# ysnrkdm/subproc

Measured on AMD Instinct MI355X. Metric: env-steps/sec (batched self-play), higher is better.
Workload: dtype u64

## Files before the change

### subproc_amd/csrc/othello.hip

```cpp
#include <hip/hip_runtime.h>
#include <stdint.h>
#include <stdlib.h>

#include <algorithm>
#include <climits>
#include <cmath>
#include <atomic>
#include <mutex>

#include "../../include/othello.h"
#include "bitboard.hpp"
#include "td_skey.hpp"

#define OTH_VERSION "subproc_amd 0.1.0 gfx950"

namespace {

using namespace oth;

constexpr u64 OPEN_BLACK = 0x0000000810000000ull;
constexpr u64 OPEN_WHITE = 0x0000001008000000ull;
constexpr int kBlock = 256;

constexpr u64 GOLDEN64 = 0x9E3779B97F4A7C15ull;
__host__ __device__ __forceinline__ u64 mix64(u64 z) {
    z = (z ^ (z >> 30)) * 0xBF58476D1CE4E5B9ull;
    z = (z ^ (z >> 27)) * 0x94D049BB133111EBull;
    return z ^ (z >> 31);
}
__device__ __forceinline__ u64 game_key(u64 S, u64 g) { return mix64(S + g * GOLDEN64); }
constexpr u32 LCG_MUL = 0x915F77F5u;
struct GameRng {
    u32 state, inc;
    __device__ __forceinline__ void init(u64 key) {
        state = (u32)key;
        inc = (u32)(key >> 32) | 1u;
    }
    __device__ __forceinline__ u32 pick(u32 n) {
        state = state * LCG_MUL + inc;
        return __umulhi(state, n);
    }
};
__device__ __forceinline__ u32 pick_legal(u64 legal, GameRng& rng, const uint8_t* kth_tab) {
    const u32 c_lo = __popc((u32)legal);
    return kth_bit_tab(legal, rng.pick(c_lo + __popc((u32)(legal >> 32))), c_lo, kth_tab);
}


__constant__ u64 kRegionMasks[8] = {0x8100000000000081ull, 0x4281000000008142ull, 0x0042000000004200ull,
                                    0x2400810000810024ull, 0x1800008181000018ull, 0x003C424242423C00ull,
                                    0x0000240000240000ull, 0x0000183C3C180000ull};

constexpr int kEvalRow = 12;
constexpr int kEvalTable = OTH_EVAL_PHASES * kEvalRow;
struct EvalWeights {
    int8_t w[OTH_EVAL_WEIGHTS];
};
__device__ __forceinline__ u32 eval_shard(u32 discs) { return discs ? (min(discs, 64u) - 1u) >> 4 : 0u; }
__device__ __forceinline__ void eval_weights_to_lds(const EvalWeights& ew, int* w_s) {
    for (int e = threadIdx.x; e < OTH_EVAL_PHASES * kEvalRow; e += blockDim.x) {
        const int r = e / kEvalRow, c = e % kEvalRow;
        w_s[e] = c < OTH_EVAL_FEATURES ? (int)ew.w[r * OTH_EVAL_FEATURES + c] : 0;
    }
}
__device__ __forceinline__ int eval_mul(int w, int c) { return __mul24(w, c); }
__device__ __forceinline__ int eval_linear(const int* w, u64 mine, u64 mob) {
    int v = eval_mul(w[0], (int)__popcll(mob));
#pragma unroll
    for (int k = 0; k < 8; k++) v += eval_mul(w[1 + k], (int)__popcll(and2(mine, kRegionMasks[k])));
    return v;
}

template <int POLICY>
__device__ __forceinline__ const int* child_row(u64 P, u64 O, const int* w_tab) {
    if (POLICY != OTH_POLICY_EVAL) return w_tab;
    return w_tab + kEvalRow * eval_shard((u32)__popcll(P | O) + 1u);
}
template <int POLICY>
__device__ __forceinline__ u32 child_key(u64 P, u64 O, const RunSets& s, u32 sq, const u64* rays, const int* row) {
    place(P, O, flips_rays(sq, s, rays));
    if (POLICY == OTH_POLICY_GREEDY) return ((u32)__popcll(moves(O, P)) << 6) | sq;
    int w[OTH_EVAL_FEATURES];
#pragma unroll
    for (int j = 0; j < OTH_EVAL_FEATURES; j++) w[j] = row[j];
    const int v = eval_linear(w, P, moves<789>(P, O));
    return ((u32)((1 << 20) - v) << 6) | sq;
}

template <int POLICY>
__device__ __forceinline__ u32 lane_choose(const Position& pos, u64 P, u64 O, const u64* rays, const int* w_tab) {
    u32 best = 0xFFFFFFFFu;
    u64 legal = pos.legal;
    const RunSets s = run_sets_parent(P, pos);
    const int* row = child_row<POLICY>(P, O, w_tab);
    while (legal) {
        const u32 sq = (u32)__builtin_ctzll(legal);
        legal &= legal - 1;
        best = min(best, child_key<POLICY>(P, O, s, sq, rays, row));
    }
    return best & 63u;
}

struct CoopWave {
    u64 rec[64][10];
    u64 legal[64];
    u32 best[64];
};
__device__ __forceinline__ void wave_sync() {
    __builtin_amdgcn_fence(__ATOMIC_SEQ_CST, "wavefront");
    __builtin_amdgcn_wave_barrier();
}
static_assert(sizeof(Runs) == 8 * sizeof(u64), "parent record: P, O, Runs");
__device__ __forceinline__ void load_parent(const u64* r, u64& P, u64& O, RunSets& s) {
    P = r[0];
    O = r[1];
    s.r = *reinterpret_cast<const Runs*>(r + 2);
    s.P = P;
    s.rP = 0;
}
__device__ __forceinline__ u32 wave_incl_scan(u32 x) {
    x += (u32)__builtin_amdgcn_update_dpp(0, (int)x, 0x111, 0xf, 0xf, false);
    x += (u32)__builtin_amdgcn_update_dpp(0, (int)x, 0x112, 0xf, 0xf, false);
    x += (u32)__builtin_amdgcn_update_dpp(0, (int)x, 0x114, 0xf, 0xf, false);
    x += (u32)__builtin_amdgcn_update_dpp(0, (int)x, 0x118, 0xf, 0xf, false);
    x += (u32)__builtin_amdgcn_update_dpp(0, (int)x, 0x142, 0xa, 0xf, false);
    x += (u32)__builtin_amdgcn_update_dpp(0, (int)x, 0x143, 0xc, 0xf, false);
    return x;
}
template <int POLICY>
__device__ u32 coop_choose(bool need, u64 P, u64 O, u32 tbl, const Position& pos, CoopWave& cw, const u64* rays,
                           const int* w_s, const uint8_t* kth_tab, u32 lane, u32 cap) {
    auto publish = [&] {
        u64* r = cw.rec[lane];
        r[0] = P;
        r[1] = O;
        Runs rs = run_sets_parent(P, pos).r;
        if (POLICY == OTH_POLICY_EVAL) rs.A1 |= (u64)(tbl & 1u);
        *reinterpret_cast<Runs*>(r + 2) = rs;
    };
    constexpr bool kFirst = POLICY == OTH_POLICY_GREEDY;
    if (kFirst && need) publish();
    if (cap == 0) return need ? lane_choose<POLICY>(pos, P, O, rays, w_s + (tbl ? kEvalTable : 0)) : 64u;
    const u64 legal = need ? pos.legal : 0ull;
    const u32 cnt = (u32)__popcll(legal);
    const u32 incl = wave_incl_scan(cnt);
    const u32 T = (u32)__builtin_amdgcn_readlane((int)incl, 63);
    const u32 R = (T + 63u) >> 6;
    cw.legal[lane] = legal;
    if (need) {
        if (!kFirst) publish();
        cw.best[lane] = 0xFFFFFFFFu;
    }
    const u32 t0 = R * lane, cnt_mine = t0 < T ? min(R, T - t0) : 0u;
    const u32 excl = incl - cnt;
    const u64 with_moves = __ballot(cnt != 0);
    u32 p = 0;
#pragma unroll
    for (u32 step = 32; step >= 1; step >>= 1)
        if ((u32)__shfl((int)excl, (int)(p + step)) <= t0) p += step;
    const u32 k0 = t0 - (u32)__shfl((int)excl, (int)p);
    wave_sync();
    u64 m = 0, Pp = 0, Op = 0;
    RunSets ps = {};
    const int* row = w_s;
// ... 72 lines not shown
    if (o.ret >= 0) o.t = black ? OTH_WHITE : OTH_BLACK;
    return o;
}

__global__ __launch_bounds__(kBlock) void legal_kernel(const u64* __restrict__ boards,
                                                       const uint8_t* __restrict__ turn, u64* __restrict__ legal,
                                                       int64_t n) {
    const int64_t i = (int64_t)blockIdx.x * kBlock + threadIdx.x;
    if (i >= n) return;
    const ulonglong2 b = reinterpret_cast<const ulonglong2*>(boards)[i];
    legal[i] = legal_any(b.x, b.y, turn[i]);
}

__device__ __forceinline__ void step_board(int64_t i, ulonglong2 b, u32 t, u32 mvc, u64* boards_out, uint8_t* turn_out,
                                           u64* __restrict__ flips_out,
                                           u64* __restrict__ legal_next, int8_t* __restrict__ ret_out,
                                           uint8_t* __restrict__ nturn) {
    u64 nb, nw, f = 0, lg = 0;
    u32 t_out;
    int r = -1;
    if (t == OTH_BLACK || t == OTH_WHITE) {
        const bool black = t == OTH_BLACK;
        u64 P = black ? b.x : b.y;
        u64 O = black ? b.y : b.x;
        if (mvc == OTH_PASS) {
            r = 0;
        } else if (mvc < 64) {
            const u64 mv = 1ull << mvc;
            if (!((P | O) & mv)) {
                f = flips_carry(mvc, P, O);
                if (f) {
                    r = __popcll(f);
                    P = or3(P, f, mv);
                    O = andn(O, f);
                }
            }
        }
        const bool moved = r >= 0;
        t_out = moved ? (t ^ 3u) : t;
        if (legal_next) {
            const u64 nP = moved ? O : P, nO = moved ? P : O;
            lg = moves(nP, nO);
        }
        nb = black ? P : O;
        nw = black ? O : P;
    } else {
        const StepOut o = put_s_any(b.x, b.y, t, mvc);
        nb = o.bl;
        nw = o.wh;
        f = o.flips;
        r = o.ret;
        t_out = o.t;
        if (legal_next) lg = legal_any(nb, nw, t_out);
    }
    if (legal_next) __builtin_nontemporal_store(lg, legal_next + i);
    if (boards_out) {
        __builtin_nontemporal_store(nb, boards_out + 2 * i);
        __builtin_nontemporal_store(nw, boards_out + 2 * i + 1);
    }
    if (turn_out) __builtin_nontemporal_store((uint8_t)t_out, turn_out + i);
    if (flips_out) __builtin_nontemporal_store(f, flips_out + i);
    if (ret_out) __builtin_nontemporal_store((int8_t)r, ret_out + i);
    if (nturn && r >= 0) nturn[i] = (uint8_t)(nturn[i] + 1);
}

constexpr int kStepPerThread = 1;
__global__ __launch_bounds__(kBlock) void step_kernel(const u64* boards_in, const uint8_t* turn_in,
                                                      const uint8_t* __restrict__ move, u64* boards_out,
                                                      uint8_t* turn_out, u64* __restrict__ flips_out,
                                                      u64* __restrict__ legal_next, int8_t* __restrict__ ret_out,
                                                      uint8_t* __restrict__ nturn, int64_t n) {
    const int64_t i0 = (int64_t)blockIdx.x * kBlock + threadIdx.x, stride = (int64_t)gridDim.x * kBlock;
    ulonglong2 b[kStepPerThread];
    u32 t[kStepPerThread], mvc[kStepPerThread];
#pragma unroll
    for (int j = 0; j < kStepPerThread; j++) {
        const int64_t i = i0 + j * stride;
        if (i < n) {
            b[j] = reinterpret_cast<const ulonglong2*>(boards_in)[i];
            t[j] = turn_in[i];
            mvc[j] = move[i];
            asm volatile("" ::"v"(t[j]), "v"(mvc[j]));
        }
    }
#pragma unroll
    for (int j = 0; j < kStepPerThread; j++) {
        const int64_t i = i0 + j * stride;
        if (i < n) step_board(i, b[j], t[j], mvc[j], boards_out, turn_out, flips_out, legal_next, ret_out, nturn);
    }
}

__device__ __forceinline__ bool step_on_board(int64_t x, int64_t d, int k, int64_t& out) {
    int64_t t;
    return !__builtin_mul_overflow(d, (int64_t)k, &t) && !__builtin_add_overflow(x, t, &out) && out >= 0 && out < 8;
}
__global__ __launch_bounds__(kBlock) void hands_kernel(const u64* __restrict__ own, const u64* __restrict__ hostile,
                                                       const int64_t* __restrict__ xs, const int64_t* __restrict__ ys,
                                                       const int64_t* __restrict__ dxs,
                                                       const int64_t* __restrict__ dys,
                                                       uint8_t* __restrict__ count, int64_t n) {
    const int64_t i = (int64_t)blockIdx.x * kBlock + threadIdx.x;
    if (i >= n) return;
    const u64 mine = own[i], opp = hostile[i];
    const int64_t x = xs[i], y = ys[i], dx = dxs[i], dy = dys[i];
    int run = 0;
    for (int k = 1; k < 9; k++) {
        int64_t nx, ny;
        const bool on = step_on_board(x, dx, k, nx) && step_on_board(y, dy, k, ny);
        const u64 bit = on ? 1ull << (nx + 8 * ny) : 0ull;
        if (opp & bit) {
            run = k;
        } else {
            if (!(mine & bit)) run = 0;
            break;
        }
    }
    count[i] = (uint8_t)run;
}

__global__ __launch_bounds__(kBlock) void result_kernel(const u64* __restrict__ boards, uint8_t* __restrict__ nb,
                                                        uint8_t* __restrict__ nw, int8_t* __restrict__ diff,
                                                        uint8_t* __restrict__ terminal, int64_t n) {
    const int64_t i = (int64_t)blockIdx.x * kBlock + threadIdx.x;
    if (i >= n) return;
    const ulonglong2 b = reinterpret_cast<const ulonglong2*>(boards)[i];
    const int cb = __popcll(b.x), cw = __popcll(b.y);
    if (nb) nb[i] = (uint8_t)cb;
    if (nw) nw[i] = (uint8_t)cw;
    if (diff) diff[i] = (int8_t)(cb - cw);
    if (terminal) terminal[i] = (moves(b.x, b.y) == 0 && moves(b.y, b.x) == 0) ? 1 : 0;
}


struct RolloutArgs {
    const u64* start;
    const uint8_t* start_turn;
    u64 seed_state;
    u64 game_id0;
    int n_random;
    u64* final_boards;
    int8_t* diff;
    uint8_t* plies;
    uint8_t* moves;
    long long* hist;
    int64_t n;
    unsigned long long* work;
    u64 last_ticket;
    u32 coop_cap;
    EvalWeights ew[2];
    u32 n_rand_a, n_rand_b;
    int swap;
    uint8_t* a_black;
    u32 handoff_k;
};

constexpr u32 kHandoffK = 16;
constexpr u32 kHandoffKMax = 16;
constexpr int kPoolCap = 64 + (int)kHandoffKMax;
struct Parked {
    u64 P, O;
    u32 state, inc;
    u32 g;
    u32 bits;
};
static_assert(sizeof(Parked) == 32, "two 16-B LDS accesses per parked game");
constexpr u64 kParkedGame = ~0ull;

constexpr int kRecStride = OTH_MOVES_STRIDE + 4;
constexpr int kRecWaveBytes = 64 * kRecStride;
constexpr size_t rec_stage_bytes(int policy, bool record) {
    return record && policy == OTH_POLICY_RANDOM ? (size_t)(kBlock / 64) * kRecWaveBytes : 0;
}

constexpr int kRandomFillOrder = 789;
constexpr int rollout_waves_per_simd(int policy) { return policy == OTH_POLICY_GREEDY ? 5 : 4; }
template <int POLICY, bool RECORD, bool RUNNER = false>
__global__ __launch_bounds__(kBlock, rollout_waves_per_simd(POLICY)) void rollout_kernel(RolloutArgs a) {
    __shared__ unsigned long long hist_s[OTH_HIST_BINS];
    __shared__ uint8_t kth_tab[256 * 8];
    __shared__ u64 rays[kTabRows * 64];
    __shared__ int w_s[POLICY == OTH_POLICY_EVAL ? 2 * kEvalTable : 1];
    __shared__ CoopWave coop[POLICY == OTH_POLICY_RANDOM ? 1 : kBlock / 64];
    constexpr bool kPool = POLICY == OTH_POLICY_RANDOM && !RECORD && !RUNNER;
    __shared__ Parked pool_s[kPool ? kBlock / 64 : 1][kPool ? kPoolCap : 1];
    for (int k = threadIdx.x; k < OTH_HIST_BINS; k += kBlock) hist_s[k] = 0;
    kth_table_init(kth_tab);
    ray_table_init(rays);
    if (POLICY == OTH_POLICY_EVAL) {
        eval_weights_to_lds(a.ew[0], w_s);
        eval_weights_to_lds(a.ew[1], w_s + kEvalTable);
    }
    __syncthreads();

    const int lane = lane_id();
    const u64 n = (u64)a.n;
    u64 plies_sum = 0;
    constexpr bool kRecStage = RECORD && POLICY == OTH_POLICY_RANDOM;
    extern __shared__ u32 rec_dyn[];
    uint8_t* const rec_wave = reinterpret_cast<uint8_t*>(rec_dyn) + (threadIdx.x >> 6) * kRecWaveBytes;
    uint8_t* const rec_row = rec_wave + lane * kRecStride;

    Parked* const pool = pool_s[kPool ? threadIdx.x >> 6 : 0];
    u32 parked = 0;
    bool exhausted = false;
    (void)pool;
    (void)exhausted;
    for (;;) {
        bool from_pool = false;
        u64 base = 0;
        if (kPool && parked >= 64u) {
            from_pool = true;
        } else if (!kPool || !exhausted) {
            if (lane == 0) {
                base = atomicAdd(a.work, 64ull);
                if (base == a.last_ticket) atomicExch(a.work, 0ull);
            }
            base = __shfl(base, 0);
            if (base >= n) {
                if (!kPool || parked == 0u) break;
                exhausted = true;
                from_pool = true;
            }
        } else {
            if (parked == 0u) break;
            from_pool = true;
        }

        u64 g = base + lane;
        bool active = !from_pool && g < n;
        u64 P = OPEN_BLACK, O = OPEN_WHITE;
        u32 side = OTH_BLACK, ply = 0;
        bool passed = false;
        GameRng rng;
        if (active) {
            rng.init(game_key(a.seed_state, a.game_id0 + g));
            if (a.start) {
                const ulonglong2 s0 = reinterpret_cast<const ulonglong2*>(a.start)[g];
                side = a.start_turn ? a.start_turn[g] : OTH_BLACK;
                side = side == OTH_WHITE ? OTH_WHITE : OTH_BLACK;
                P = side == OTH_BLACK ? s0.x : s0.y;
                O = side == OTH_BLACK ? s0.y : s0.x;
            }
            if (RECORD && !kRecStage) {
                uint4* mrec = reinterpret_cast<uint4*>(a.moves + g * OTH_MOVES_STRIDE);
#pragma unroll
                for (int q = 0; q < OTH_MOVES_STRIDE / 16; q++) mrec[q] = make_uint4(~0u, ~0u, ~0u, ~0u);
            }
        }
        if constexpr (kRecStage) {
#pragma unroll
            for (int q = 0; q < OTH_MOVES_STRIDE / 4; q++) reinterpret_cast<u32*>(rec_row)[q] = ~0u;
        }
        auto rec_put = [&](u32 i, uint8_t code) {
            if (i >= OTH_MOVES_STRIDE) return;
            if constexpr (kRecStage) rec_row[i] = code;
            else a.moves[g * OTH_MOVES_STRIDE + i] = code;
        };

        if constexpr (POLICY == OTH_POLICY_RANDOM) {
            bool b0 = side == OTH_BLACK;
            u32 discs0 = RECORD ? 0u : (u32)__popcll(P | O);
            u32 npass = 0;
            if (kPool && from_pool) {
                const u32 take = min(parked, 64u);
                active = (u32)lane < take;
                if (active) {
                    const Parked e = pool[parked - take + lane];
                    P = e.P;
                    O = e.O;
                    rng.state = e.state;
                    rng.inc = e.inc;
                    g = e.g;
                    b0 = e.bits & 1u;
                    passed = (e.bits >> 1) & 1u;
                    discs0 = (e.bits >> 2) & 0x7fu;
                    npass = e.bits >> 9;
                }
                parked -= take;
            }
            const u32 hand_k = __builtin_amdgcn_readfirstlane(kPool && !from_pool ? a.handoff_k : 0u);
            const u32 parked0 = __builtin_amdgcn_readfirstlane(parked);
            (void)hand_k;
            (void)parked0;
            auto ply_of = [&](u64& X, u64& Y) -> bool {
                Position pos;
                analyse<kRandomFillOrder>(X, Y, pos);
                const u64 legal = pos.legal;
                const u32 c_lo = __popc((u32)legal), nl = c_lo + __popc((u32)(legal >> 32));
                if (nl == 0) {
                    if (passed || (X | Y) == ~0ull) {
                        if (passed) npass--;
                        return true;
                    }
                    if (RECORD) rec_put(npass, OTH_PASS);
                    passed = true;
                    npass++;
                    return false;
                }
                passed = false;
                const u32 off = kth_bit_off(legal, rng.pick(nl), c_lo, kth_tab);
                const u64* col = ray_col(rays, off);
                const Flips f = flips_col(col[kRayRows * 64], run_sets(X, pos), col);
                if (RECORD) {
                    rec_put(npass, (uint8_t)(off >> 3));
                    npass++;
                }
                place(X, Y, f);
                return false;
            };
            if (active) {
                for (;;) {
                    if (ply_of(P, O)) break;
                    if (ply_of(O, P)) break;
                    if (kPool) {
                        const u64 live = __ballot(1);
                        if ((u32)__popcll(live) <= hand_k) {
                            const u32 rank = __builtin_amdgcn_mbcnt_hi((u32)(live >> 32),
                                                                       __builtin_amdgcn_mbcnt_lo((u32)live, 0u));
                            pool[parked0 + rank] = Parked{P, O, rng.state, rng.inc, (u32)g,
                                                          (u32)b0 | (u32)passed << 1 | discs0 << 2 | npass << 9};
                            g = kParkedGame;
                            break;
                        }
                    }
                }
            }
            if (kPool) {
                const u64 pm = __ballot(active && g == kParkedGame);
                parked = parked0 + (u32)__popcll(pm);
                if (g == kParkedGame) active = false;
            }
            if (active) {
                const u32 ply = RECORD ? npass : (u32)__popcll(P | O) - discs0 + npass;
                if (RECORD) rec_put(ply, 0xFF);
                const u64 bl = b0 ? P : O, wh = b0 ? O : P;
                const int d = __popcll(bl) - __popcll(wh);
                if (a.final_boards) reinterpret_cast<ulonglong2*>(a.final_boards)[g] = make_ulonglong2(bl, wh);
                if (a.diff) a.diff[g] = (int8_t)d;
                if (a.plies) a.plies[g] = (uint8_t)ply;
                atomicAdd(&hist_s[d + 64], 1ull);
                atomicAdd(&hist_s[d > 0 ? 129 : (d < 0 ? 130 : 131)], 1ull);
                plies_sum += ply;
            }
        } else {
            u32 rem_b = 0, rem_w = 0, tbl_black = 0;
            if (RUNNER && active) {
                const bool ab = !(a.swap && rng.pick(2) == 1u);
                rem_b = ab ? a.n_rand_a : a.n_rand_b;
                rem_w = ab ? a.n_rand_b : a.n_rand_a;
                tbl_black = ab ? 0u : 1u;
                if (a.a_black) a.a_black[g] = (uint8_t)ab;
            }
            while (__ballot(active)) {
                bool moving = false, choose = false;
                u32 sq = 0;
                Position pos;
                if (active) {
                    analyse(P, O, pos);
                    const u64 legal = pos.legal;
                    if (legal == 0) {
                        if (passed || (P | O) == ~0ull) {
                            const u64 bl = side == OTH_BLACK ? P : O, wh = side == OTH_BLACK ? O : P;
                            const int d = __popcll(bl) - __popcll(wh);
                            u64 gt = g;
                            if (POLICY == OTH_POLICY_GREEDY) asm volatile("" : "+v"(gt));
                            if (a.final_boards)
                                reinterpret_cast<ulonglong2*>(a.final_boards)[gt] = make_ulonglong2(bl, wh);
                            if (a.diff) a.diff[gt] = (int8_t)d;
                            if (a.plies) a.plies[gt] = (uint8_t)ply;
                            atomicAdd(&hist_s[d + 64], 1ull);
                            atomicAdd(&hist_s[d > 0 ? 129 : (d < 0 ? 130 : 131)], 1ull);
                            if (POLICY == OTH_POLICY_GREEDY) atomicAdd(&hist_s[132], (unsigned long long)ply);
                            else plies_sum += ply;
                            active = false;
                        } else {
                            passed = true;
                            const u64 t = P;
                            P = O;
                            O = t;
                            side ^= 3u;
                        }
                    } else {
                        if (passed) {
                            if (RECORD) rec_put(ply, OTH_PASS);
                            ply++;
                            passed = false;
                            if (RUNNER) {
                                const u32 rx = side == OTH_BLACK ? rem_w : rem_b;
                                if (rx) (void)rng.pick(rx);
                            }
                        }
                        moving = true;
                        if (RUNNER) {
                            const u32 r = side == OTH_BLACK ? rem_b : rem_w;
                            if (r && rng.pick(r) == 0u) {
                                sq = pick_legal(legal, rng, kth_tab);
                                if (side == OTH_BLACK) rem_b--;
                                else rem_w--;
                            } else {
                                choose = true;
                            }
                        } else if ((int)ply >= a.n_random) {
                            choose = true;
                        } else {
                            sq = pick_legal(legal, rng, kth_tab);
                        }
                    }
                }
                CoopWave& cw = coop[__builtin_amdgcn_readfirstlane(threadIdx.x >> 6)];
                auto play = [&](u32 m, const RunSets& rs) {
                    if (RECORD) rec_put(ply, (uint8_t)m);
                    place(P, O, flips_rays(m, rs, rays));
                    const u64 np = O;
                    O = P;
                    P = np;
                    side ^= 3u;
                    ply++;
                };
                constexpr bool kFromRecord = POLICY == OTH_POLICY_GREEDY;
                if (kFromRecord && moving && !choose) play(sq, run_sets_parent(P, pos));
                if (__ballot(choose)) {
                    const u32 tbl = side == OTH_BLACK ? tbl_black : tbl_black ^ 1u;
                    const u32 c = coop_choose<POLICY>(choose, P, O, tbl, pos, cw, rays, w_s, kth_tab, (u32)lane,
                                                      a.coop_cap);
                    if (choose) {
                        sq = c;
                        if (kFromRecord) {
                            u64 Pr, Or;
                            RunSets rs;
                            load_parent(cw.rec[lane], Pr, Or, rs);
                            play(c, rs);
// ... 853 lines not shown
                if (miss) {
                    g = pred;
                    f = w;
                }
            }
            prev = __shfl(f, (int)min<int64_t>(kSpecLanes - 1, np - 1 - c0));
        }
        if (lane == 0) out[s] = prev;
    }
}
inline size_t spec_scratch_bytes(int64_t n_long, int64_t n_values) {
    const int64_t parts = n_values / kSpecLen + n_long + 1;
    return sizeof(int64_t) * kSpecHdr + sizeof(SpecPlanEntry) * (size_t)std::max<int64_t>(n_long, 1) +
           2 * sizeof(double) * (size_t)parts;
}

constexpr int kTdStage = 512;
constexpr int kTdStageLoads = kTdStage / 64;
struct LongStage {
    double stage[2][kTdStage], ystage[2][kTdStage + kTdChunk];
};
__device__ __forceinline__ void td_ema_long_body(int64_t blk, const double* __restrict__ vals,
                                                 const int64_t* __restrict__ seg_off,
                                                 const double* __restrict__ init, double a, double oma,
                                                 double* __restrict__ out, const int64_t* __restrict__ long_idx,
                                                 int64_t warm, LongStage& ls) {
    double(&stage)[2][kTdStage] = ls.stage;
    double(&ystage)[2][kTdStage + kTdChunk] = ls.ystage;
    const int lane = threadIdx.x;
    const int64_t s = long_idx[blk];
    const int64_t b = seg_off[s], e = seg_off[s + 1];
    if (warm > 0 && e - b >= kSpecMinWarms * warm && e - b <= kSpecMaxLen) return;
    const int64_t n_stage = (e - b + kTdStage - 1) / kTdStage;
    double r[kTdStageLoads];
    auto fetch = [&](int64_t c) {
#pragma unroll
        for (int k = 0; k < kTdStageLoads; k++) {
            const int64_t idx = b + c * kTdStage + k * 64 + lane;
            r[k] = idx < e ? vals[idx] : 0.0;
        }
    };
    auto park = [&](int buf) {
#pragma clang fp contract(off)
#pragma unroll
        for (int k = 0; k < kTdStageLoads; k++) {
            stage[buf][k * 64 + lane] = r[k];
            ystage[buf][k * 64 + lane] = r[k] * a;
        }
    };
    fetch(0);
    park(0);
    __syncthreads();
    double v = (lane == 0 && init) ? init[s] : 0.0;
    for (int64_t c = 0; c < n_stage; c++) {
        if (c + 1 < n_stage) fetch(c + 1);
        if (lane == 0) {
            const double* x = stage[c & 1];
            const double* y = ystage[c & 1];
            const int m = (int)min<int64_t>(kTdStage, e - b - c * kTdStage);
            auto chunk = [&](const double(&yk)[kTdChunk], int j0) {
                double w = v, mn = 1.0;
#pragma unroll
                for (int k = 0; k < kTdChunk; k++) {
                    double t;
                    asm("v_mul_f64 %[t], %[w], %[oma]\n\t"
                        "v_min_f64 %[mn], %[mn], |%[w]|\n\t"
                        "v_add_f64 %[w], %[t], %[y]"
                        : [w] "+v"(w), [mn] "+v"(mn), [t] "=&v"(t)
                        : [oma] "v"(oma), [y] "v"(yk[k]));
                }
                if (mn == 0.0) {
                    double bk[kTdChunk];
#pragma unroll
                    for (int k = 0; k < kTdChunk; k++) bk[k] = x[j0 + k];
                    w = td_run(v, bk, kTdChunk, a, oma);
                }
                v = w;
            };
            double ya[kTdChunk], yb[kTdChunk];
            auto load = [&](double(&yk)[kTdChunk], int j0) {
#pragma unroll
                for (int k = 0; k < kTdChunk; k++) yk[k] = y[j0 + k];
            };
            int j = 0;
            load(ya, 0);
            for (; j + 2 * kTdChunk <= m; j += 2 * kTdChunk) {
                load(yb, j + kTdChunk);
                chunk(ya, j);
                load(ya, j + 2 * kTdChunk);
                chunk(yb, j + kTdChunk);
            }
            if (j + kTdChunk <= m) {
                chunk(ya, j);
                j += kTdChunk;
            }
            double bk[kTdChunk];
#pragma unroll
            for (int k = 0; k < kTdChunk; k++) bk[k] = x[min(j + k, kTdStage - 1)];
            v = td_run(v, bk, m - j, a, oma);
        }
        if (c + 1 < n_stage) park((c + 1) & 1);
        __syncthreads();
    }
    if (lane == 0) out[s] = v;
}
__global__ __launch_bounds__(64) void td_ema_long_kernel(const double* __restrict__ vals,
                                                         const int64_t* __restrict__ seg_off,
                                                         const double* __restrict__ init, double a, double oma,
                                                         double* __restrict__ out,
                                                         const int64_t* __restrict__ long_idx, int64_t warm) {
    __shared__ LongStage ls;
    td_ema_long_body(blockIdx.x, vals, seg_off, init, a, oma, out, long_idx, warm, ls);
}
union LongOrParts {
    LongStage ls;
    SpecWave sw;
};
__global__ __launch_bounds__(64) void td_ema_long_parts_kernel(const double* __restrict__ vals,
                                                               const int64_t* __restrict__ seg_off,
                                                               const double* __restrict__ init, double a, double oma,
                                                               double* __restrict__ out,
                                                               const int64_t* __restrict__ long_idx, int64_t warm,
                                                               int64_t n_long, const int64_t* __restrict__ hdr,
                                                               const SpecPlanEntry* __restrict__ plan,
                                                               double* __restrict__ guess, double* __restrict__ fin,
                                                               int warm16, int64_t parts_grid) {
    __shared__ LongOrParts lp;
    const int64_t blk = blockIdx.x;
    if (blk < parts_grid)
        td_spec_parts_body(blk, parts_grid, vals, seg_off, init, a, oma, hdr, plan, guess, fin, warm16, lp.sw);
    else
        td_ema_long_body(blk - parts_grid, vals, seg_off, init, a, oma, out, long_idx, warm, lp.ls);
}

inline int status(hipError_t e) { return e == hipSuccess ? OTH_OK : -(int)e; }

struct Tuning {
    unsigned resident_blocks[3];
    unsigned random_big_blocks;
};

int env_int(const char* name, int dflt) {
    const char* v = getenv(name);
    return v && *v ? atoi(v) : dflt;
}

constexpr int kMaxDevices = 64;
constexpr int kMaxBlocksPerCu = 5;
constexpr int kRandomBlocksPerCu = 3;
constexpr int64_t kBigLaunch = 1 << 22;
struct DeviceState {
    std::atomic<int> ready{0};
    Tuning tuning;
};
DeviceState g_dev[kMaxDevices];
std::mutex g_dev_mu;

DeviceState* device_state() {
    int dev = 0;
    (void)hipGetDevice(&dev);
    if (dev < 0 || dev >= kMaxDevices) return nullptr;
    DeviceState& d = g_dev[dev];
    if (d.ready.load(std::memory_order_acquire)) return &d;
    std::lock_guard<std::mutex> lock(g_dev_mu);
    if (!d.ready.load(std::memory_order_relaxed)) {
        int cus = 256;
        (void)hipDeviceGetAttribute(&cus, hipDeviceAttributeMultiprocessorCount, dev);
        const void* kern[3] = {reinterpret_cast<const void*>(rollout_kernel<OTH_POLICY_RANDOM, false>),
                               reinterpret_cast<const void*>(rollout_kernel<OTH_POLICY_GREEDY, false>),
                               reinterpret_cast<const void*>(rollout_kernel<OTH_POLICY_EVAL, false>)};
        for (int p = 0; p < 3; p++) {
            int per_cu = 0;
            (void)hipOccupancyMaxActiveBlocksPerMultiprocessor(&per_cu, kern[p], kBlock, 0);
            const int occ = per_cu;
            const int cap = p == OTH_POLICY_RANDOM ? kRandomBlocksPerCu : kMaxBlocksPerCu;
            per_cu = occ > 0 ? std::min(occ, cap) : 2;
            per_cu = env_int("OTH_ROLLOUT_BLOCKS_PER_CU", per_cu);
            d.tuning.resident_blocks[p] = (unsigned)(cus * per_cu);
            if (p == OTH_POLICY_RANDOM) {
                const int big = env_int("OTH_ROLLOUT_BLOCKS_PER_CU", occ > 0 ? std::min(occ, kMaxBlocksPerCu) : 2);
                d.tuning.random_big_blocks = (unsigned)(cus * big);
            }
        }
        d.ready.store(1, std::memory_order_release);
    }
    return &d;
}
inline unsigned blocks_for(int64_t n) { return (unsigned)((n + kBlock - 1) / kBlock); }
inline int launched() { return status(hipGetLastError()); }
static int td_updates_launch(const u64* pos, const int64_t* row_off, const uint8_t* plies, const int64_t* base,
                             const double* lam_pow, int64_t* keys, double* vals, u64* words, int64_t n, hipStream_t s) {
    (words ? td_updates_wave_kernel<true> : td_updates_wave_kernel<false>)<<<
        blocks_for((n + kTdUpdGames - 1) / kTdUpdGames * 64), kBlock, 0, s>>>(pos, row_off, plies, base, lam_pow, keys,
                                                                               vals, words, n);
    return launched();
}

}

extern "C" {

const char* oth_version(void) { return OTH_VERSION; }

int oth_reset(uint64_t* boards, uint8_t* turn, uint8_t* nturn, int64_t n, void* stream) {
    if (n < 0 || (n > 0 && !boards)) return OTH_EINVAL;
    if (n == 0) return OTH_OK;
    reset_kernel<<<blocks_for(n), kBlock, 0, (hipStream_t)stream>>>(boards, turn, nturn, n);
    return launched();
}

int oth_legal(const uint64_t* boards, const uint8_t* turn, uint64_t* legal, int64_t n, void* stream) {
    if (n < 0 || (n > 0 && (!boards || !turn || !legal))) return OTH_EINVAL;
    if (n == 0) return OTH_OK;
    legal_kernel<<<blocks_for(n), kBlock, 0, (hipStream_t)stream>>>(boards, turn, legal, n);
    return launched();
}

int oth_step(const uint64_t* boards_in, const uint8_t* turn_in, const uint8_t* move, uint64_t* boards_out,
             uint8_t* turn_out, uint64_t* flips, uint64_t* legal_next, int8_t* ret, uint8_t* nturn, int64_t n,
             void* stream) {
    if (n < 0 || (n > 0 && (!boards_in || !turn_in || !move))) return OTH_EINVAL;
    if (n == 0) return OTH_OK;
    step_kernel<<<blocks_for((n + kStepPerThread - 1) / kStepPerThread), kBlock, 0, (hipStream_t)stream>>>(
        boards_in, turn_in, move, boards_out, turn_out, flips, legal_next, ret, nturn, n);
    return launched();
}

int oth_hands(const uint64_t* own, const uint64_t* hostile, const int64_t* x, const int64_t* y, const int64_t* dx,
              const int64_t* dy, uint8_t* count, int64_t n, void* stream) {
    if (n < 0 || (n > 0 && (!own || !hostile || !x || !y || !dx || !dy || !count))) return OTH_EINVAL;
    if (n == 0) return OTH_OK;
    hands_kernel<<<blocks_for(n), kBlock, 0, (hipStream_t)stream>>>(own, hostile, x, y, dx, dy, count, n);
    return launched();
}

int oth_result(const uint64_t* boards, uint8_t* n_black, uint8_t* n_white, int8_t* diff, uint8_t* terminal,
               int64_t n, void* stream) {
    if (n < 0 || (n > 0 && !boards)) return OTH_EINVAL;
    if (n == 0) return OTH_OK;
    result_kernel<<<blocks_for(n), kBlock, 0, (hipStream_t)stream>>>(boards, n_black, n_white, diff, terminal, n);
    return launched();
}

namespace {
struct RunnerSpec {
    int n_rand_a, n_rand_b, swap;
    uint8_t* a_black;
};
int rollout_launch(const uint64_t* start, const uint8_t* start_turn, uint64_t seed, uint64_t game_id0, int policy,
                   int n_random, const int8_t* w_black, const int8_t* w_white, uint64_t* final_boards, int8_t* diff,
                   uint8_t* plies, uint8_t* moves, int64_t* hist, uint64_t* work, int64_t n, void* stream,
                   const RunnerSpec* run = nullptr) {
    RolloutArgs a;
    a.n_rand_a = run ? (u32)std::min(run->n_rand_a, 10) : 0u;
    a.n_rand_b = run ? (u32)std::min(run->n_rand_b, 10) : 0u;
    a.swap = run ? run->swap : 0;
    a.a_black = run ? run->a_black : nullptr;
    a.start = start;
    a.start_turn = start_turn;
    a.seed_state = mix64(seed + GOLDEN64);
    a.game_id0 = game_id0;
    a.n_random = n_random;
    a.final_boards = final_boards;
    a.diff = diff;
    a.plies = plies;
    a.moves = moves;
    a.hist = (long long*)hist;
    a.n = n;
    for (int k = 0; k < OTH_EVAL_WEIGHTS; k++) {
        a.ew[0].w[k] = w_black ? w_black[k] : 0;
        a.ew[1].w[k] = w_white ? w_white[k] : 0;
    }
    DeviceState* ds = device_state();
    if (!ds) return status(hipErrorInvalidDevice);
    const Tuning& t = ds->tuning;
    const int64_t max_blocks = (n + kBlock - 1) / kBlock;
    const unsigned resident =
        policy == OTH_POLICY_RANDOM && n >= kBigLaunch ? t.random_big_blocks : t.resident_blocks[policy];
    const unsigned grid = (unsigned)std::min<int64_t>(max_blocks, (int64_t)resident);
    a.work = reinterpret_cast<unsigned long long*>(work);
    a.coop_cap = env_int("OTH_COOP_CAP", 1) == 0 ? 0u : 1u;
    a.last_ticket = 64ull * ((u64)((n + 63) / 64) + (u64)grid * (kBlock / 64) - 1ull);
    a.handoff_k = n <= 0xFFFFFFFFll
                      ? (u32)std::min(std::max(env_int("OTH_HANDOFF_K", (int)kHandoffK), 0), (int)kHandoffKMax)
                      : 0u;
    hipStream_t st = (hipStream_t)stream;
    if (run) {
        if (policy == OTH_POLICY_EVAL) {
            if (moves) rollout_kernel<OTH_POLICY_EVAL, true, true><<<grid, kBlock, 0, st>>>(a);
            else rollout_kernel<OTH_POLICY_EVAL, false, true><<<grid, kBlock, 0, st>>>(a);
        } else {
            if (moves) rollout_kernel<OTH_POLICY_GREEDY, true, true><<<grid, kBlock, 0, st>>>(a);
            else rollout_kernel<OTH_POLICY_GREEDY, false, true><<<grid, kBlock, 0, st>>>(a);
        }
    } else if (policy == OTH_POLICY_EVAL) {
        if (moves) rollout_kernel<OTH_POLICY_EVAL, true><<<grid, kBlock, 0, st>>>(a);
        else rollout_kernel<OTH_POLICY_EVAL, false><<<grid, kBlock, 0, st>>>(a);
    } else if (policy == OTH_POLICY_GREEDY) {
        if (moves) rollout_kernel<OTH_POLICY_GREEDY, true><<<grid, kBlock, 0, st>>>(a);
        else rollout_kernel<OTH_POLICY_GREEDY, false><<<grid, kBlock, 0, st>>>(a);
    } else {
        if (moves)
            rollout_kernel<OTH_POLICY_RANDOM, true><<<grid, kBlock, rec_stage_bytes(OTH_POLICY_RANDOM, true), st>>>(a);
        else rollout_kernel<OTH_POLICY_RANDOM, false><<<grid, kBlock, 0, st>>>(a);
    }
    return launched();
}
}

int oth_rollout(const uint64_t* start, const uint8_t* start_turn, uint64_t seed, uint64_t game_id0, int policy,
                int n_random, uint64_t* final_boards, int8_t* diff, uint8_t* plies, uint8_t* moves, int64_t* hist,
                uint64_t* work, int64_t n, void* stream) {
    if (n < 0 || !work || (policy != OTH_POLICY_RANDOM && policy != OTH_POLICY_GREEDY)) return OTH_EINVAL;
    if (n == 0) return OTH_OK;
    return rollout_launch(start, start_turn, seed, game_id0, policy, n_random, nullptr, nullptr, final_boards, diff,
                          plies, moves, hist, work, n, stream);
}

int oth_rollout_eval(const uint64_t* start, const uint8_t* start_turn, uint64_t seed, uint64_t game_id0,
                     int n_random, const int8_t* weights, uint64_t* final_boards, int8_t* diff, uint8_t* plies,
                     uint8_t* moves, int64_t* hist, uint64_t* work, int64_t n, void* stream) {
    if (n < 0 || !weights || !work) return OTH_EINVAL;
    if (n == 0) return OTH_OK;
    return rollout_launch(start, start_turn, seed, game_id0, OTH_POLICY_EVAL, n_random, weights, weights, final_boards,
                          diff, plies, moves, hist, work, n, stream);
}

int oth_rollout_match(const uint64_t* start, const uint8_t* start_turn, uint64_t seed, uint64_t game_id0,
                      int n_random, const int8_t* weights_black, const int8_t* weights_white, uint64_t* final_boards,
                      int8_t* diff, uint8_t* plies, uint8_t* moves, int64_t* hist, uint64_t* work, int64_t n,
                      void* stream) {
    if (n < 0 || !weights_black || !weights_white || !work) return OTH_EINVAL;
    if (n == 0) return OTH_OK;
    return rollout_launch(start, start_turn, seed, game_id0, OTH_POLICY_EVAL, n_random, weights_black, weights_white,
                          final_boards, diff, plies, moves, hist, work, n, stream);
}

int oth_rollout_runner(const uint64_t* start, const uint8_t* start_turn, uint64_t seed, uint64_t game_id0, int policy,
                       const int8_t* weights_a, const int8_t* weights_b, int n_rand_a, int n_rand_b, int swap_colours,
                       uint8_t* a_black, uint64_t* final_boards, int8_t* diff, uint8_t* plies, uint8_t* moves,
                       int64_t* hist, uint64_t* work, int64_t n, void* stream) {
    if (n < 0 || !work || (policy != OTH_POLICY_GREEDY && policy != OTH_POLICY_EVAL) ||
        (policy == OTH_POLICY_EVAL && (!weights_a || !weights_b)) || n_rand_a < 0 || n_rand_b < 0)
        return OTH_EINVAL;
    if (n == 0) return OTH_OK;
    const RunnerSpec run{n_rand_a, n_rand_b, swap_colours != 0, a_black};
    return rollout_launch(start, start_turn, seed, game_id0, policy, 0, weights_a, weights_b, final_boards, diff,
                          plies, moves, hist, work, n, stream, &run);
}

int oth_replay(const uint64_t* start, const uint8_t* start_turn, const uint8_t* moves, const uint8_t* plies,
               uint64_t* pos_boards, uint8_t* pos_turn, uint8_t* pos_end, int64_t n, void* stream) {
    if (n < 0 || (n > 0 && (!moves || !plies || !pos_boards))) return OTH_EINVAL;
    if (n == 0) return OTH_OK;
    const bool staged = pos_turn || pos_end;
    const int vec_moves = ((uintptr_t)moves & 15) == 0;
    const int vec_out = (((uintptr_t)pos_turn | (uintptr_t)pos_end) & 15) == 0;
    replay_kernel<false><<<blocks_for(n), kBlock, staged ? kReplayStage : 0, (hipStream_t)stream>>>(
        start, start_turn, moves, plies, nullptr, pos_boards, pos_turn, pos_end, n, vec_moves, vec_out);
    return launched();
}

int oth_replay_rows(const uint64_t* start, const uint8_t* start_turn, const uint8_t* moves, const uint8_t* plies,
                    const int64_t* row_off, uint64_t* pos_boards, uint8_t* pos_turn, uint8_t* pos_end, int64_t n,
                    void* stream) {
    if (n < 0 || (n > 0 && (!moves || !plies || !row_off || !pos_boards))) return OTH_EINVAL;
    if (n == 0) return OTH_OK;
    const bool staged = pos_turn || pos_end;
    const int vec_moves = ((uintptr_t)moves & 15) == 0;
    const int vec_out = (((uintptr_t)pos_turn | (uintptr_t)pos_end) & 15) == 0;
    replay_kernel<true><<<blocks_for(n), kBlock, staged ? kReplayStagePacked : 0, (hipStream_t)stream>>>(
        start, start_turn, moves, plies, row_off, pos_boards, pos_turn, pos_end, n, vec_moves, vec_out);
    return launched();
}


int oth_book_text(const uint64_t* boards, const uint8_t* turn, int64_t n, char* out, void* stream) {
    if (n < 0 || (n > 0 && (!boards || !turn || !out))) return OTH_EINVAL;
    if (n == 0) return OTH_OK;
    book_text_kernel<<<blocks_for(n), kBlock, 0, (hipStream_t)stream>>>(boards, turn, n,
                                                                       reinterpret_cast<uint8_t*>(out),
                                                                       ((uintptr_t)out & 15) == 0);
    return launched();
}

int oth_book_parse(const char* text, int64_t stride, uint64_t* boards, uint8_t* turn, int64_t n, void* stream) {
    if (n < 0 || stride < 64 || (turn && stride < 66) || (n > 0 && (!text || !boards))) return OTH_EINVAL;
    if (n == 0) return OTH_OK;
    const int vec = ((uintptr_t)text & 15) == 0 && stride % 16 == 0;
    book_parse_kernel<<<blocks_for(n), kBlock, 0, (hipStream_t)stream>>>(reinterpret_cast<const uint8_t*>(text),
                                                                        stride, boards, turn, n, vec);
    return launched();
}

int oth_features(const uint64_t* boards, const uint8_t* side, uint8_t* out, int64_t n, void* stream) {
    if (n < 0 || (n > 0 && (!boards || !side || !out))) return OTH_EINVAL;
    if (n == 0) return OTH_OK;
    features_kernel<<<blocks_for(n), kBlock, 0, (hipStream_t)stream>>>(boards, side, out, n);
    return launched();
}

int oth_eval(const uint64_t* boards, const uint8_t* side, const int8_t* weights, int32_t* out, int64_t n,
             void* stream) {
    if (n < 0 || !weights || (n > 0 && (!boards || !side || !out))) return OTH_EINVAL;
    if (n == 0) return OTH_OK;
    EvalWeights ew;
    for (int k = 0; k < OTH_EVAL_WEIGHTS; k++) ew.w[k] = weights[k];
    eval_kernel<<<blocks_for(n), kBlock, 0, (hipStream_t)stream>>>(boards, side, ew, out, n);
    return launched();
}

int oth_td_updates(const uint64_t* pos_boards, const uint8_t* plies, const int64_t* base, const double* lam_pow,
                   int64_t* keys, double* values, int64_t n, void* stream) {
    if (n < 0 || (n > 0 && (!pos_boards || !plies || !base || !lam_pow || !keys || !values))) return OTH_EINVAL;
    if (n == 0) return OTH_OK;
    return td_updates_launch(pos_boards, nullptr, plies, base, lam_pow, keys, values, nullptr, n, (hipStream_t)stream);
}

int oth_td_updates_packed(const uint64_t* pos_boards, const int64_t* row_off, const uint8_t* plies,
                          const int64_t* base, uint64_t* words, int64_t n, void* stream) {
    if (n < 0 || (n > 0 && (!pos_boards || !plies || !base || !words))) return OTH_EINVAL;
    if (n == 0) return OTH_OK;
    return td_updates_launch(pos_boards, row_off, plies, base, nullptr, nullptr, nullptr, reinterpret_cast<u64*>(words),
                             n, (hipStream_t)stream);
}
int oth_td_updates_rows(const uint64_t* pos_boards, const int64_t* row_off, const uint8_t* plies, const int64_t* base,
                        const double* lam_pow, int64_t* keys, double* values, int64_t n, void* stream) {
    if (n < 0 || (n > 0 && (!pos_boards || !row_off || !plies || !base || !lam_pow || !keys || !values)))
        return OTH_EINVAL;
    if (n == 0) return OTH_OK;
    return td_updates_launch(pos_boards, row_off, plies, base, lam_pow, keys, values, nullptr, n, (hipStream_t)stream);
}

int oth_td_updates_records(const uint64_t* rows, const int64_t* term_row, const int32_t* lam_idx,
                           const double* lam_pow, int64_t* keys, double* values, int64_t n_rows, void* stream) {
    if (n_rows < 0 || (n_rows > 0 && (!rows || !term_row || !lam_idx || !lam_pow || !keys || !values)))
        return OTH_EINVAL;
    if (n_rows == 0) return OTH_OK;
    td_records_kernel<<<blocks_for(n_rows), kBlock, 0, (hipStream_t)stream>>>(rows, term_row, lam_idx, lam_pow, keys,
                                                                              values, n_rows);
    return launched();
}

int oth_td_ema(const double* values, const int64_t* seg_off, const double* init, double a, double one_minus_a,
               double* out, int64_t n_seg, void* stream) {
    if (n_seg < 0 || (n_seg > 0 && (!values || !seg_off || !out))) return OTH_EINVAL;
    if (n_seg == 0) return OTH_OK;
    td_ema_kernel<false><<<blocks_for(n_seg), kBlock, 0, (hipStream_t)stream>>>(values, seg_off, init, a,
                                                                                one_minus_a, out, n_seg, 0);
    return launched();
}

struct TdSides {
    std::mutex mu;
    bool made = false;
    int rc = OTH_OK;
    hipStream_t side[2] = {nullptr, nullptr};
// ... 147 lines not shown
```

Measured before the change: 224.2 billion.

## Sample random-rollout openings from a precomputed device-side opening tree

Builds, once per device, a tree of every position reachable in the first plies from the standard Othello start, stored in device memory. The upper levels and the leaf boards are staged into dynamic LDS. Random-policy rollouts with no caller-supplied start position then walk the tree with their RNG instead of generating and playing the first moves, which removes move generation for those opening plies. The cost is extra LDS per block, which may lower occupancy, a changed RNG stream and a one-time host-synchronous build that is skipped during stream capture.

```diff
diff --git a/subproc_amd/csrc/opening_tree.hpp b/subproc_amd/csrc/opening_tree.hpp
--- /dev/null
+++ b/subproc_amd/csrc/opening_tree.hpp
@@ -0,0 +1,95 @@
+#pragma once
+#include <hip/hip_runtime.h>
+#include <stdint.h>
+
+#include "bitboard.hpp"
+
+namespace oth {
+
+constexpr int kOpeningDepthMax = 8;
+constexpr u32 kOpeningLevel[kOpeningDepthMax + 1] = {1, 4, 12, 56, 244, 1396, 8200, 55092, 390216};
+constexpr u32 opening_off(int d) {
+    u32 s = 0;
+    for (int i = 0; i < d; i++) s += kOpeningLevel[i];
+    return s;
+}
+constexpr u32 kOpeningInternal = opening_off(kOpeningDepthMax);
+constexpr u32 kOpeningNodes = opening_off(kOpeningDepthMax + 1);
+static_assert(kOpeningInternal == 65005u && kOpeningNodes == 455221u, "level sizes");
+constexpr u32 kOpeningErrNoMove = 1u, kOpeningErrOverflow = 2u, kOpeningErrWide = 4u;
+constexpr u32 kOpeningNlBits = 5u, kOpeningNlMask = (1u << kOpeningNlBits) - 1u;
+static_assert(kOpeningNodes < (1u << (32u - kOpeningNlBits)), "child_base fits its field");
+constexpr int kOpeningLdsDepth = 6;
+constexpr int kOpeningLdsLeafDepth = 4;
+constexpr size_t opening_lds_bytes(int depth) {
+    return (depth > 0 && depth <= kOpeningLdsLeafDepth ? kOpeningLevel[depth] * sizeof(ulonglong2) : 0) +
+           (depth > 0 ? opening_off(depth < kOpeningLdsDepth ? depth : kOpeningLdsDepth) * sizeof(u32) : 0);
+}
+
+struct OpeningTree {
+    ulonglong2* boards;
+    u32* nodes;
+    u32* count;
+};
+constexpr size_t kOpeningBoardsBytes = (size_t)kOpeningNodes * sizeof(ulonglong2);
+constexpr size_t kOpeningNodesBytes = (size_t)kOpeningInternal * sizeof(u32);
+constexpr size_t kOpeningCountBytes = (kOpeningDepthMax + 2) * sizeof(u32);
+constexpr size_t kOpeningBytes = kOpeningBoardsBytes + kOpeningNodesBytes + kOpeningCountBytes;
+inline OpeningTree opening_tree_at(void* base) {
+    char* p = static_cast<char*>(base);
+    return OpeningTree{reinterpret_cast<ulonglong2*>(p), reinterpret_cast<u32*>(p + kOpeningBoardsBytes),
+                       reinterpret_cast<u32*>(p + kOpeningBoardsBytes + kOpeningNodesBytes)};
+}
+
+__global__ void opening_root_kernel(OpeningTree t, u64 mover, u64 other) {
+    if (blockIdx.x == 0 && threadIdx.x == 0) {
+        t.boards[0] = make_ulonglong2(mover, other);
+        t.count[0] = 1u;
+    }
+}
+
+__global__ __launch_bounds__(256) void opening_level_kernel(OpeningTree t, int d, u32 off, u32 off_next, u32 end_next) {
+    const u32 i = blockIdx.x * blockDim.x + threadIdx.x;
+    if (i >= t.count[d] || i >= off_next - off) return;
+    const ulonglong2 b = t.boards[off + i];
+    const u64 P = b.x, O = b.y;
+    u64 legal = moves(P, O);
+    const u32 nl = (u32)__popcll(legal);
+    if (nl == 0u || nl > kOpeningNlMask) {
+        atomicOr(&t.count[kOpeningDepthMax + 1], nl ? kOpeningErrWide : kOpeningErrNoMove);
+        return;
+    }
+    const u32 base = off_next + atomicAdd(&t.count[d + 1], nl);
+    if (base < off_next || base > end_next || nl > end_next - base) {
+        atomicOr(&t.count[kOpeningDepthMax + 1], kOpeningErrOverflow);
+        return;
+    }
+    t.nodes[off + i] = base << kOpeningNlBits | nl;
+    for (u32 k = 0; k < nl; k++) {
+        const u32 sq = (u32)__ffsll((long long)legal) - 1u;
+        legal &= legal - 1ull;
+        const u64 f = flips_carry(sq, P, O);
+        t.boards[base + k] = make_ulonglong2(O & ~f, P | f | (1ull << sq));
+    }
+}
+
+inline bool opening_tree_build(void* base, u64 open_mover, u64 open_other, hipStream_t s) {
+    const OpeningTree t = opening_tree_at(base);
+    if (hipMemsetAsync(t.count, 0, kOpeningCountBytes, s) != hipSuccess) return false;
+    opening_root_kernel<<<1, 64, 0, s>>>(t, open_mover, open_other);
+    for (int d = 0; d < kOpeningDepthMax; d++) {
+        const u32 n = kOpeningLevel[d];
+        opening_level_kernel<<<(n + 255u) / 256u, 256, 0, s>>>(t, d, opening_off(d), opening_off(d + 1),
+                                                              opening_off(d + 2));
+    }
+    u32 count[kOpeningDepthMax + 2] = {};
+    if (hipMemcpyAsync(count, t.count, kOpeningCountBytes, hipMemcpyDeviceToHost, s) != hipSuccess) return false;
+    if (hipStreamSynchronize(s) != hipSuccess) return false;
+    if (hipGetLastError() != hipSuccess) return false;
+    if (count[kOpeningDepthMax + 1] != 0u) return false;
+    for (int d = 0; d <= kOpeningDepthMax; d++)
+        if (count[d] != kOpeningLevel[d]) return false;
+    return true;
+}
+
+}
diff --git a/subproc_amd/csrc/othello.hip b/subproc_amd/csrc/othello.hip
--- a/subproc_amd/csrc/othello.hip
+++ b/subproc_amd/csrc/othello.hip
@@ -10,6 +10,7 @@
 
 #include "../../include/othello.h"
 #include "bitboard.hpp"
+#include "opening_tree.hpp"
 #include "td_skey.hpp"
 
 #define OTH_VERSION "subproc_amd 0.1.0 gfx950"
@@ -388,6 +389,12 @@
     int swap;
     uint8_t* a_black;
     u32 handoff_k;
+    u32 open_depth;
+    u32 open_lds_nodes;
+    u32 open_lds_leaves;
+    u32 open_leaf0;
+    const u32* open_nodes;
+    const ulonglong2* open_boards;
 };
 
 constexpr u32 kHandoffK = 16;
@@ -419,6 +426,14 @@
     __shared__ CoopWave coop[POLICY == OTH_POLICY_RANDOM ? 1 : kBlock / 64];
     constexpr bool kPool = POLICY == OTH_POLICY_RANDOM && !RECORD && !RUNNER;
     __shared__ Parked pool_s[kPool ? kBlock / 64 : 1][kPool ? kPoolCap : 1];
+    extern __shared__ ulonglong2 open_dyn[];
+    ulonglong2* const open_leaf_s = open_dyn;
+    u32* const open_s = reinterpret_cast<u32*>(open_dyn + (kPool ? a.open_lds_leaves : 0u));
+    if (kPool && a.open_depth) {
+        for (u32 k = threadIdx.x; k < a.open_lds_leaves; k += kBlock)
+            open_leaf_s[k] = a.open_boards[a.open_leaf0 + k];
+        for (u32 k = threadIdx.x; k < a.open_lds_nodes; k += kBlock) open_s[k] = a.open_nodes[k];
+    }
     for (int k = threadIdx.x; k < OTH_HIST_BINS; k += kBlock) hist_s[k] = 0;
     kth_table_init(kth_tab);
     ray_table_init(rays);
@@ -513,6 +528,26 @@
                     npass = e.bits >> 9;
                 }
                 parked -= take;
+            }
+            if constexpr (kPool) {
+                const u32 depth = __builtin_amdgcn_readfirstlane(from_pool ? 0u : a.open_depth);
+                if (depth && active) {
+                    u32 node = 0;
+                    const u32 in_lds = min(depth, (u32)kOpeningLdsDepth);
+                    for (u32 d = 0; d < in_lds; d++) {
+                        const u32 e = open_s[node];
+                        node = (e >> kOpeningNlBits) + rng.pick(e & kOpeningNlMask);
+                    }
+                    for (u32 d = in_lds; d < depth; d++) {
+                        const u32 e = a.open_nodes[node];
+                        node = (e >> kOpeningNlBits) + rng.pick(e & kOpeningNlMask);
+                    }
+                    const ulonglong2 leaf =
+                        a.open_lds_leaves ? open_leaf_s[node - a.open_leaf0] : a.open_boards[node];
+                    P = leaf.x;
+                    O = leaf.y;
+                    b0 = !(depth & 1u);
+                }
             }
             const u32 hand_k = __builtin_amdgcn_readfirstlane(kPool && !from_pool ? a.handoff_k : 0u);
             const u32 parked0 = __builtin_amdgcn_readfirstlane(parked);
@@ -1672,9 +1707,43 @@
 struct DeviceState {
     std::atomic<int> ready{0};
     Tuning tuning;
+    std::atomic<void*> tree{nullptr};
+    bool tree_failed = false;
 };
 DeviceState g_dev[kMaxDevices];
 std::mutex g_dev_mu;
+
+constexpr int kOpeningDepth = 4;
+
+void* opening_tree(DeviceState& d, hipStream_t caller) {
+    if (void* t = d.tree.load(std::memory_order_acquire)) return t;
+    hipStreamCaptureStatus cap = hipStreamCaptureStatusNone;
+    if (hipStreamIsCapturing(caller, &cap) != hipSuccess || cap != hipStreamCaptureStatusNone) {
+        (void)hipGetLastError();
+        return nullptr;
+    }
+    std::lock_guard<std::mutex> lock(g_dev_mu);
+    if (void* t = d.tree.load(std::memory_order_relaxed)) return t;
+    if (d.tree_failed) return nullptr;
+    void* base = nullptr;
+    hipStream_t s = nullptr;
+    bool ok = hipMalloc(&base, kOpeningBytes) == hipSuccess;
+    if (ok) {
+        ok = hipStreamCreateWithFlags(&s, hipStreamNonBlocking) == hipSuccess;
+        if (ok) {
+            ok = opening_tree_build(base, OPEN_BLACK, OPEN_WHITE, s);
+            (void)hipStreamDestroy(s);
+        }
+        if (!ok) (void)hipFree(base);
+    }
+    (void)hipGetLastError();
+    if (!ok) {
+        d.tree_failed = true;
+        return nullptr;
+    }
+    d.tree.store(base, std::memory_order_release);
+    return base;
+}
 
 DeviceState* device_state() {
     int dev = 0;
@@ -1805,6 +1874,25 @@
                       ? (u32)std::min(std::max(env_int("OTH_HANDOFF_K", (int)kHandoffK), 0), (int)kHandoffKMax)
                       : 0u;
     hipStream_t st = (hipStream_t)stream;
+    a.open_depth = a.open_lds_nodes = a.open_lds_leaves = a.open_leaf0 = 0u;
+    size_t open_lds = 0;
+    a.open_nodes = nullptr;
+    a.open_boards = nullptr;
+    if (policy == OTH_POLICY_RANDOM && !run && !moves && !start) {
+        const int depth = std::min(std::max(env_int("OTH_OPENING_DEPTH", kOpeningDepth), 0), kOpeningDepthMax);
+        if (depth > 0) {
+            if (void* base = opening_tree(*ds, st)) {
+                const OpeningTree tree = opening_tree_at(base);
+                a.open_depth = (u32)depth;
+                a.open_lds_nodes = opening_off(std::min(depth, kOpeningLdsDepth));
+                a.open_lds_leaves = depth <= kOpeningLdsLeafDepth ? kOpeningLevel[depth] : 0u;
+                a.open_leaf0 = opening_off(depth);
+                open_lds = opening_lds_bytes(depth);
+                a.open_nodes = tree.nodes;
+                a.open_boards = tree.boards;
+            }
+        }
+    }
     if (run) {
         if (policy == OTH_POLICY_EVAL) {
             if (moves) rollout_kernel<OTH_POLICY_EVAL, true, true><<<grid, kBlock, 0, st>>>(a);
@@ -1822,7 +1910,7 @@
     } else {
         if (moves)
             rollout_kernel<OTH_POLICY_RANDOM, true><<<grid, kBlock, rec_stage_bytes(OTH_POLICY_RANDOM, true), st>>>(a);
-        else rollout_kernel<OTH_POLICY_RANDOM, false><<<grid, kBlock, 0, st>>>(a);
+        else rollout_kernel<OTH_POLICY_RANDOM, false><<<grid, kBlock, open_lds, st>>>(a);
     }
     return launched();
 }
```

New measurement: 235.1 billion, median of 6. 4.9% higher.
